# alanqrwang/nwhead

Hardware: AMD Instinct MI355X
Metric: query-predictions/sec (higher is better)
Workload: dtype f32; 1 GPU; K3 predict('full'): B=256 queries/step vs bank N=50000 d=512 C=200, bank sharded 1-way, 26 query batches coalesced per launch; B=256, N_support=50000, d=512, C=200, parallelism=support-shard x1

## Files before the change

nwhead_amd/csrc/fused_f16p.h:

```cpp
#pragma once
#include "fused_impl.h"
#include "persistent_pipe.h"

namespace nw {
namespace {

template <int RS, int QB, bool TWO = false>
struct PCfg : PipeCfg<16 * RS, 64 * QB, NCONS, NLOAD, TWO ? 3 : 4> {};

template <int RS, int KIND, int QB, int NCW = NCONS>
__device__ __forceinline__ void epilogue_p(f32x4 (&acc)[QB][RS], const float* hdr, int nrun, int2 bnd,
                                           const float* __restrict__ logit_scale, float* __restrict__ ws_m,
                                           float* __restrict__ ws_den, float* __restrict__ ws_num, int B, int N,
                                           int q0, int s0, int st, int wave, int lane
#ifdef NW_DIAG_FUSED
                                           , unsigned long long (&diag_)[8], unsigned long long& last_
#endif
                                           ) {
    using P = PCfg<RS, QB>;
    constexpr int BS = P::BS;
    constexpr bool NEED_NORM = (KIND != NW_SCORE_DOT);
    constexpr float L2E = 1.44269504088896340736f;
    typedef float f32x2 __attribute__((ext_vector_type(2)));
    const float* sn2 = hdr;
    const float* ssc = hdr + P::NH;
    const int* runid = reinterpret_cast<const int*>(hdr + 2 * P::NH);
    const float* qn2 = hdr + 3 * P::NH;
    const float* qsc_s = qn2 + 16 * QB * NCW;
    const int i = lane & 15, g = lane >> 4;
    float scale = 1.f;
    if (KIND == NW_SCORE_CLIP) scale = expf(*logit_scale);
    using SF = ScoreFactors<KIND>;
    float4 n4[RS], s4[RS];
#pragma unroll
    for (int r = 0; r < RS; ++r) {
        n4[r] = NEED_NORM ? *reinterpret_cast<const float4*>(sn2 + 16 * r + 4 * g) : make_float4(0.f, 0.f, 0.f, 0.f);
        s4[r] = *reinterpret_cast<const float4*>(ssc + 16 * r + 4 * g);
    }
    NW_PSTAMP(1);
    float4 K4[RS], B4[RS];
#pragma unroll
    for (int r = 0; r < RS; ++r) {
        SF::support(n4[r].x, s4[r].x, K4[r].x, B4[r].x);
        SF::support(n4[r].y, s4[r].y, K4[r].y, B4[r].y);
        SF::support(n4[r].z, s4[r].z, K4[r].z, B4[r].z);
        SF::support(n4[r].w, s4[r].w, K4[r].w, B4[r].w);
    }
#pragma unroll
    for (int j = 0; j < QB; ++j) {
        const int qrow = 16 * (QB * wave + j) + i;
        const int b = q0 + qrow;
        float Cq, Bq;
        SF::query(NEED_NORM ? qn2[qrow] : 0.f, qsc_s[qrow], scale, Cq, Bq);
        const f32x2 cq = {Cq, Cq}, bq = {Bq, Bq};
        float sc[RS][4];
#pragma unroll
        for (int r = 0; r < RS; ++r) {
            const f32x2 d01 = __builtin_elementwise_fma(f32x2{acc[j][r][0], acc[j][r][1]}, f32x2{K4[r].x, K4[r].y} * cq,
                                                        f32x2{B4[r].x, B4[r].y} + bq);
            const f32x2 d23 = __builtin_elementwise_fma(f32x2{acc[j][r][2], acc[j][r][3]}, f32x2{K4[r].z, K4[r].w} * cq,
                                                        f32x2{B4[r].z, B4[r].w} + bq);
            sc[r][0] = SF::finish_abs(d01.x);
            sc[r][1] = SF::finish_abs(d01.y);
            sc[r][2] = SF::finish_abs(d23.x);
            sc[r][3] = SF::finish_abs(d23.y);
        }
        NW_PSTAMP(2);
        constexpr float WORST = SF::DIST ? INFINITY : -INFINITY;
        if (s0 + BS > N) {
#pragma unroll
            for (int r = 0; r < RS; ++r)
#pragma unroll
                for (int e = 0; e < 4; ++e)
                    if (s0 + 16 * r + 4 * g + e >= N) sc[r][e] = WORST;
        }
        auto best = [](float a, float b) { return SF::DIST ? fminf(a, b) : fmaxf(a, b); };
        float mx[4] = {WORST, WORST, WORST, WORST};
#pragma unroll
        for (int r = 0; r < RS; ++r) mx[r & 3] = best(mx[r & 3], best(best(sc[r][0], sc[r][1]), best(sc[r][2], sc[r][3])));
        float ext = best(best(mx[0], mx[1]), best(mx[2], mx[3]));
        ext = SF::DIST ? group4_min(ext) : group4_max(ext);
        const float mloc = SF::DIST ? -ext : ext;
#pragma unroll
        for (int r = 0; r < RS; ++r)
#pragma unroll
            for (int e = 0; e < 4; ++e)
                sc[r][e] = __builtin_amdgcn_exp2f(SF::DIST ? ext - sc[r][e] : sc[r][e] - ext);
        NW_PSTAMP(3);
        float dloc;
        auto red4 = [](float x) { return group4_sum(x); };
        if (nrun <= 3) {
            float S0[2] = {0.f, 0.f}, S1[2] = {0.f, 0.f}, S2[2] = {0.f, 0.f};
            if (nrun == 1) {
#pragma unroll
                for (int r = 0; r < RS; ++r) {
                    S0[r & 1] += (sc[r][0] + sc[r][1]) + (sc[r][2] + sc[r][3]);
                }
            } else {
                const int b1 = bnd.x, b2 = (nrun == 3) ? bnd.y : BS;
                const float L1 = (float)(b1 - 4 * g);
                const float M2 = 1.f - (float)(b2 - 4 * g);
#pragma unroll
                for (int r = 0; r < RS; ++r) {
                    const int lo = 16 * r, hi = 16 * r + 16;
                    const bool in0 = hi <= b1, in2 = lo >= b2, in1 = lo >= b1 && hi <= b2;
                    const float quad = (sc[r][0] + sc[r][1]) + (sc[r][2] + sc[r][3]);
                    S0[r & 1] = __builtin_fmaf(in0 ? 1.f : 0.f, quad, S0[r & 1]);
                    S1[r & 1] = __builtin_fmaf(in1 ? 1.f : 0.f, quad, S1[r & 1]);
                    S2[r & 1] = __builtin_fmaf(in2 ? 1.f : 0.f, quad, S2[r & 1]);
                    if (!(in0 || in1 || in2)) {
#pragma unroll
                        for (int e = 0; e < 4; ++e) {
                            const float c = (float)(16 * r + e), ev = sc[r][e];
                            const float w1 = __builtin_amdgcn_fmed3f(L1 - c, 0.f, 1.f);
                            const float u2 = __builtin_amdgcn_fmed3f(c + M2, 0.f, 1.f);
                            S0[e & 1] = __builtin_fmaf(w1, ev, S0[e & 1]);
                            S2[e & 1] = __builtin_fmaf(u2, ev, S2[e & 1]);
                            S1[e & 1] = __builtin_fmaf((1.f - w1) - u2, ev, S1[e & 1]);
                        }
                    }
                }
            }
            const float s0v = red4(S0[0] + S0[1]);
            float s1v = 0.f, s2v = 0.f;
            if (nrun >= 2) s1v = red4(S1[0] + S1[1]);
            if (nrun == 3) s2v = red4(S2[0] + S2[1]);
            dloc = (s0v + s1v) + s2v;
            if (g == 0 && b < B) {
                ws_num[((size_t)st * BS) * B + b] = s0v;
                if (nrun >= 2) ws_num[((size_t)st * BS + 1) * B + b] = s1v;
                if (nrun == 3) ws_num[((size_t)st * BS + 2) * B + b] = s2v;
            }
        } else {
            float dl[4] = {0.f, 0.f, 0.f, 0.f};
#pragma unroll
            for (int r = 0; r < RS; ++r) dl[r & 3] += (sc[r][0] + sc[r][1]) + (sc[r][2] + sc[r][3]);
            dloc = red4((dl[0] + dl[1]) + (dl[2] + dl[3]));
            for (int run_base = 0; run_base < nrun; run_base += 16) {
                f32x4 Pm = {0.f, 0.f, 0.f, 0.f};
                const int want = run_base + i;
#pragma unroll
                for (int r = 0; r < RS; ++r) {
                    const int4 rid = *reinterpret_cast<const int4*>(runid + 16 * r + 4 * g);
                    Pm = __builtin_amdgcn_mfma_f32_16x16x4f32(rid.x == want ? 1.f : 0.f, sc[r][0], Pm, 0, 0, 0);
                    Pm = __builtin_amdgcn_mfma_f32_16x16x4f32(rid.y == want ? 1.f : 0.f, sc[r][1], Pm, 0, 0, 0);
                    Pm = __builtin_amdgcn_mfma_f32_16x16x4f32(rid.z == want ? 1.f : 0.f, sc[r][2], Pm, 0, 0, 0);
                    Pm = __builtin_amdgcn_mfma_f32_16x16x4f32(rid.w == want ? 1.f : 0.f, sc[r][3], Pm, 0, 0, 0);
                }
                if (b < B) {
#pragma unroll
                    for (int jj = 0; jj < 4; ++jj) {
                        const int run = run_base + 4 * g + jj;
                        if (run < nrun) ws_num[((size_t)st * BS + run) * B + b] = Pm[jj];
                    }
                }
            }
        }
        NW_PSTAMP(4);
        if (g == 0 && b < B) {
            ws_m[(size_t)st * B + b] = mloc;
            ws_den[(size_t)st * B + b] = dloc;
        }
        NW_PSTAMP(5);
    }
}

template <int RS, int KIND, bool TWO, int QB>
__global__ __launch_bounds__(TILE_THREADS, TWO ? 4 : 2) void nw_fused_f16p_kernel(
    const float* __restrict__ q, const float* __restrict__ s, const float* __restrict__ s_norm2,
    const float* __restrict__ s_scale, const float* __restrict__ q_norm2, const float* __restrict__ q_scale,
    const float* __restrict__ logit_scale, const int* __restrict__ ws_runid, const int* __restrict__ ws_nrun, const int* __restrict__ ws_bnd,
    float* __restrict__ ws_m, float* __restrict__ ws_den, float* __restrict__ ws_num, int B, int N, int d,
    int n_stiles, int n_qtiles, int qg) {
    using P = PCfg<RS, QB, TWO>;
    constexpr int BS = P::BS, BQP = P::BQP, TILE_F4 = P::TILE_F4, NB = P::NB;
    constexpr bool SINGLE = TWO || QB > 1;
    static_assert(!(TWO && QB > 1), "two 128-query workgroups do not fit the LDS of a CU");
    static_assert(P::THREADS == TILE_THREADS, "launch bounds");
    static_assert(RS == 8, "the persistent kernel is built for tiles of 128 supports");
    extern __shared__ __attribute__((aligned(16))) char smem[];
    float* hdr0 = reinterpret_cast<float*>(smem);
    float4* stage = reinterpret_cast<float4*>(smem + P::HDR_BYTES);

    const int tid = threadIdx.x, lane = tid & 63;
    const int wave = __builtin_amdgcn_readfirstlane(tid >> 6);
    const int nk = d / BK;
    const PersistentTiles tiles(blockIdx.x, gridDim.x, n_stiles, n_qtiles, qg);
    const int cu = tiles.cu, n_cu = tiles.n_cu, n_local = tiles.n_local;

    if (wave >= P::NCW) {
        persistent_loader<P>(tiles, wave - P::NCW, lane, hdr0, stage, q, s, s_norm2, s_scale, q_norm2, q_scale, ws_runid, B, N,
                             d);
    } else {
        const int i = lane & 15, g = lane >> 4;
        struct Frag {
            float4 bh[QB], bl[QB];
            float4 ah[RS], al[RS];
        };
        const int rsw = (i >> 1) & 7;
        auto load_frags = [&](Frag& f, int buf) {
            const float4* Qs = stage + ((unsigned)buf % NB) * TILE_F4;
            const float4* Ss = Qs + BQP * ROW_F4;
            const int sh = g ^ rsw, sl = (4 + g) ^ rsw;
#pragma unroll
            for (int j = 0; j < QB; ++j) {
                const int qrow = 16 * (QB * wave + j) + i;
                f.bh[j] = Qs[qrow * ROW_F4 + sh];
                f.bl[j] = Qs[qrow * ROW_F4 + sl];
            }
#pragma unroll
            for (int r = 0; r < RS; ++r) {
                f.ah[r] = Ss[(16 * r + i) * ROW_F4 + sh];
                f.al[r] = Ss[(16 * r + i) * ROW_F4 + sl];
            }
        };
        auto mm = [](const float4& a, const float4& b, f32x4 c) {
            return __builtin_amdgcn_mfma_f32_16x16x32_f16(__builtin_bit_cast(half8, a), __builtin_bit_cast(half8, b), c, 0, 0, 0);
        };
        f32x4 acc[QB][RS];
        auto mfma_stage = [&](const Frag& f) {
#pragma unroll
            for (int j = 0; j < QB; ++j)
#pragma unroll
                for (int r = 0; r < RS; ++r) acc[j][r] = mm(f.al[r], f.bh[j], acc[j][r]);
#pragma unroll
            for (int j = 0; j < QB; ++j)
#pragma unroll
                for (int r = 0; r < RS; ++r) acc[j][r] = mm(f.ah[r], f.bl[j], acc[j][r]);
#pragma unroll
            for (int j = 0; j < QB; ++j)
#pragma unroll
                for (int r = 0; r < RS; ++r) acc[j][r] = mm(f.ah[r], f.bh[j], acc[j][r]);
        };
        auto interleave = [&]() {
#pragma unroll
            for (int x = 0; x < 2 * (RS + 1); ++x) {
                __builtin_amdgcn_sched_group_barrier(0x008, 1, 0);
                __builtin_amdgcn_sched_group_barrier(0x100, 1, 0);
            }
            __builtin_amdgcn_sched_group_barrier(0x008, 3 * RS - 2 * (RS + 1), 0);
        };

        tile_barrier();
        int gi = 0;
        int par = 0;
#ifdef NW_DIAG_FUSED
        unsigned long long diag_[8] = {0, 0, 0, 0, 0, 0, 0, 0}, last_ = __builtin_amdgcn_s_memtime();
        const unsigned long long first_ = last_, first_rt_ = __builtin_amdgcn_s_memrealtime();
#endif
        for (int T = cu; T < n_local; T += n_cu) {
            int qt, st;
            tiles.decode(T, qt, st);
            const int q0 = qt * BQP, s0 = st * BS;
            const int nrun = ws_nrun[st];
            const int2 bnd = *reinterpret_cast<const int2*>(ws_bnd + 2 * (size_t)st);

#pragma unroll
            for (int j = 0; j < QB; ++j)
#pragma unroll
                for (int r = 0; r < RS; ++r) acc[j][r] = f32x4{0.f, 0.f, 0.f, 0.f};
            if constexpr (QB > 1) {
                struct F1 { float4 bh[QB]; float4 al[RS]; };
                struct F2 { float4 bl[QB]; float4 ah[RS]; };
                const int sh = g ^ rsw, sl = (4 + g) ^ rsw;
                const int qoff = (16 * QB * wave + i) * ROW_F4, soff = (BQP + i) * ROW_F4;
                auto stage_base = [&](int buf) { return stage + ((unsigned)buf % NB) * TILE_F4; };
                auto rd_bh = [&](const float4* S, int j) { return S[qoff + 16 * j * ROW_F4 + sh]; };
                auto rd_bl = [&](const float4* S, int j) { return S[qoff + 16 * j * ROW_F4 + sl]; };
                auto rd_ah = [&](const float4* S, int r) { return S[soff + 16 * r * ROW_F4 + sh]; };
                auto rd_al = [&](const float4* S, int r) { return S[soff + 16 * r * ROW_F4 + sl]; };
                auto pin = []() { __builtin_amdgcn_sched_barrier(0); };
                auto run_stage = [&](const F1& ac, F1& an, F2& b, int buf_next, auto has_next) {
#ifdef NW_ABL_NORD
                    constexpr bool NXT = false;
#else
                    constexpr bool NXT = decltype(has_next)::value;
#endif
                    const float4* Sn = stage_base(buf_next);
                    int n = 0;
#pragma unroll
                    for (int r = 0; r < RS; ++r)
#pragma unroll
                        for (int jx = 0; jx < QB; ++jx) {
                            const int j = (r & 1) ? QB - 1 - jx : jx;
                            acc[j][r] = mm(ac.al[r], ac.bh[j], acc[j][r]);
                            if (NXT && n < QB + RS) {
                                if (n < QB) an.bh[n] = rd_bh(Sn, n);
                                else an.al[n - QB] = rd_al(Sn, n - QB);
                            }
                            ++n;
                            pin();
                        }
#pragma unroll
                    for (int r = 0; r < RS; ++r)
#pragma unroll
                        for (int jx = 0; jx < QB; ++jx) {
                            const int j = (r & 1) ? QB - 1 - jx : jx;
                            acc[j][r] = mm(b.ah[r], b.bl[j], acc[j][r]);
                            pin();
                        }
                    if (NXT) {
#pragma unroll
                        for (int j = 0; j < QB; ++j) b.bl[j] = rd_bl(Sn, j);
                        pin();
                    }
#pragma unroll
                    for (int r = RS - 1; r >= 0; --r) {
#pragma unroll
                        for (int jx = 0; jx < QB; ++jx) {
                            const int j = (r & 1) ? jx : QB - 1 - jx;
                            acc[j][r] = mm(b.ah[r], ac.bh[j], acc[j][r]);
                        }
                        pin();
                        if (NXT) {
                            b.ah[r] = rd_ah(Sn, r);
                            pin();
                        }
                    }
                };
                using Yes = std::integral_constant<bool, true>;
                using No = std::integral_constant<bool, false>;
                F1 a0, a1;
                F2 b0;
                {
                    const float4* S0 = stage_base(gi);
#pragma unroll
                    for (int j = 0; j < QB; ++j) { a0.bh[j] = rd_bh(S0, j); b0.bl[j] = rd_bl(S0, j); }
#pragma unroll
                    for (int r = 0; r < RS; ++r) { a0.al[r] = rd_al(S0, r); b0.ah[r] = rd_ah(S0, r); }
#ifdef NW_ABL_NORD
                    a1 = a0;
#endif
                    pin();
                }
                int kt = 0;
                for (; kt + 2 < nk; kt += 2) {
                    run_stage(a0, a1, b0, gi + kt + 1, Yes{});
                    tile_barrier_nowait();
                    run_stage(a1, a0, b0, gi + kt + 2, Yes{});
                    tile_barrier_nowait();
                }
                if (kt + 2 == nk) {
                    run_stage(a0, a1, b0, gi + kt + 1, Yes{});
                    tile_barrier_nowait();
                    run_stage(a1, a0, b0, 0, No{});
                    tile_barrier_nowait();
                } else {
                    run_stage(a0, a1, b0, 0, No{});
                    tile_barrier_nowait();
                }
            } else if constexpr (SINGLE) {
                Frag f0;
                for (int kt = 0; kt < nk; ++kt) {
                    load_frags(f0, gi + kt);
                    mfma_stage(f0);
                    tile_barrier();
                }
            } else {
                Frag f0, f1;
                load_frags(f0, gi);
                int kt = 0;
                for (; kt + 2 < nk; kt += 2) {
                    load_frags(f1, gi + kt + 1);
                    mfma_stage(f0);
                    interleave();
                    tile_barrier();
                    load_frags(f0, gi + kt + 2);
                    mfma_stage(f1);
                    interleave();
                    tile_barrier();
                }
                for (; kt < nk; ++kt) {
                    if (kt + 1 < nk) load_frags(f1, gi + kt + 1);
                    mfma_stage(f0);
                    tile_barrier();
                    f0 = f1;
                }
            }
            gi += nk;
            NW_PSTAMP(0);
#ifndef NW_ABL_NOEPI
            epilogue_p<RS, KIND, QB>(acc, hdr0 + par * P::HDR_F, nrun, bnd, logit_scale, ws_m, ws_den, ws_num, B, N, q0, s0, st,
                                 wave, lane
#ifdef NW_DIAG_FUSED
                                 , diag_, last_
#endif
                                 );
#else
            keep_acc_alive(acc, ws_m, nrun, bnd);
#endif
            par = (par + 1 == P::NHB) ? 0 : par + 1;
            NW_PSTAMP(6);
        }
#ifdef NW_DIAG_FUSED
        diag_write_out(diag_, last_, first_, first_rt_);
#endif
    }
}

}
}
```

nwhead_amd/csrc/fused_f16p12.h:

```cpp
#pragma once
#include "fused_f16p.h"

namespace nw {
namespace {

struct P12 : PipeCfg<128, 256, 8, 4, 3> {
    static constexpr int RS = BS / 16, QB = BQP / (16 * NCW);
    static_assert(LDS_BYTES <= 160 * 1024, "LDS of one CU");
};

template <int KIND, bool CAND = false>
__device__ __forceinline__ void epilogue_p12(f32x4 (&acc)[P12::QB][P12::RS], const float* hdr, int nrun, int2 bnd,
                                             float scale, float* __restrict__ ws_m,
                                             float* __restrict__ ws_den, float* __restrict__ ws_num, int B, int N,
                                             int q0, int s0, int st, int wave, int lane, int n_stiles, int k
#ifdef NW_DIAG_FUSED
                                             , unsigned long long (&diag_)[8], unsigned long long& last_
#endif
                                             ) {
    using P = P12;
    constexpr int RS = P::RS, QB = P::QB, BS = P::BS;
    constexpr bool NEED_NORM = (KIND != NW_SCORE_DOT);
    typedef float f32x2 __attribute__((ext_vector_type(2)));
    const float* sn2 = hdr;
    const float* ssc = hdr + P::NH;
    const int* runid = reinterpret_cast<const int*>(hdr + 2 * P::NH);
    const float* qn2 = hdr + 3 * P::NH;
    const float* qsc_s = qn2 + P::BQP;
    const int i = lane & 15, g = lane >> 4;
    using SF = ScoreFactors<KIND>;
    float Cq[QB], Bq[QB];
#pragma unroll
    for (int j = 0; j < QB; ++j) {
        const int qrow = 16 * (QB * wave + j) + i;
        SF::query(NEED_NORM ? qn2[qrow] : 0.f, qsc_s[qrow], scale, Cq[j], Bq[j]);
    }
    NW_PSTAMP(1);
    float sc[QB][RS][4];
#pragma unroll
    for (int r = 0; r < RS; ++r) {
        const float4 n4 = NEED_NORM ? *reinterpret_cast<const float4*>(sn2 + 16 * r + 4 * g) : make_float4(0.f, 0.f, 0.f, 0.f);
        const float4 s4 = *reinterpret_cast<const float4*>(ssc + 16 * r + 4 * g);
        float4 K4, B4;
        SF::support(n4.x, s4.x, K4.x, B4.x);
        SF::support(n4.y, s4.y, K4.y, B4.y);
        SF::support(n4.z, s4.z, K4.z, B4.z);
        SF::support(n4.w, s4.w, K4.w, B4.w);
        float4 B4r = B4;
        asm volatile("" : "+v"(B4r.x), "+v"(B4r.y), "+v"(B4r.z), "+v"(B4r.w));
#pragma unroll
        for (int j = 0; j < QB; ++j) {
            const f32x2 cq = {Cq[j], Cq[j]}, bq = {Bq[j], Bq[j]};
            const float4 Bj = (j == 0) ? B4 : B4r;
            const f32x2 d01 = __builtin_elementwise_fma(f32x2{acc[j][r][0], acc[j][r][1]}, f32x2{K4.x, K4.y} * cq,
                                                        f32x2{Bj.x, Bj.y} + bq);
            const f32x2 d23 = __builtin_elementwise_fma(f32x2{acc[j][r][2], acc[j][r][3]}, f32x2{K4.z, K4.w} * cq,
                                                        f32x2{Bj.z, Bj.w} + bq);
            sc[j][r][0] = SF::finish_abs(d01.x);
            sc[j][r][1] = SF::finish_abs(d01.y);
            sc[j][r][2] = SF::finish_abs(d23.x);
            sc[j][r][3] = SF::finish_abs(d23.y);
            asm volatile("" : "+v"(sc[j][r][0]), "+v"(sc[j][r][1]), "+v"(sc[j][r][2]), "+v"(sc[j][r][3]));
        }
        __builtin_amdgcn_sched_barrier(0);
    }
    NW_PSTAMP(2);
    if constexpr (CAND) {
        int ln = lane;
        asm volatile("" : "+v"(ln));
        const int ci = ln & 15, cg = ln >> 4;
#pragma unroll
        for (int j = 0; j < QB; ++j) {
            float u[RS][4];
#pragma unroll
            for (int r = 0; r < RS; ++r)
#pragma unroll
                for (int e = 0; e < 4; ++e) u[r][e] = SF::DIST ? -sc[j][r][e] : sc[j][r][e];
            tile_candidates<RS>(u, reinterpret_cast<unsigned*>(ws_m), reinterpret_cast<int*>(ws_den), B, N,
                                q0 + 16 * (QB * wave + j) + ci, s0, cg, st, n_stiles, k);
            __builtin_amdgcn_sched_barrier(0);
        }
        return;
    }
    constexpr float WORST = SF::DIST ? INFINITY : -INFINITY;
    if (s0 + BS > N) {
        const int lim = N - s0 - 4 * g;
#pragma unroll
        for (int j = 0; j < QB; ++j)
#pragma unroll
            for (int r = 0; r < RS; ++r)
#pragma unroll
                for (int e = 0; e < 4; ++e)
                    if (16 * r + e >= lim) sc[j][r][e] = WORST;
    }
    auto best = [](float a, float b) { return SF::DIST ? fminf(a, b) : fmaxf(a, b); };
    auto best3 = [&](float a, float b, float c) { return best(best(a, b), c); };
    static_assert(RS == 8, "chain k takes the 16-row blocks k and k + 4");
    float ext[QB];
#pragma unroll
    for (int j = 0; j < QB; ++j) {
        float mx[4];
#pragma unroll
        for (int k = 0; k < 4; ++k) mx[k] = best3(sc[j][k][0], sc[j][k][1], sc[j][k][2]);
#pragma unroll
        for (int k = 0; k < 4; ++k) mx[k] = best3(mx[k], sc[j][k][3], sc[j][k + 4][0]);
#pragma unroll
        for (int k = 0; k < 4; ++k) mx[k] = best3(mx[k], sc[j][k + 4][1], sc[j][k + 4][2]);
#pragma unroll
        for (int k = 0; k < 4; ++k) mx[k] = best(mx[k], sc[j][k + 4][3]);
        ext[j] = best(best3(mx[0], mx[1], mx[2]), mx[3]);
    }
    group4_each(ext, best);
    float mloc[QB], dloc[QB], s0v[QB], s1v[QB] = {0.f, 0.f}, s2v[QB] = {0.f, 0.f};
#pragma unroll
    for (int j = 0; j < QB; ++j) {
        mloc[j] = SF::DIST ? -ext[j] : ext[j];
#pragma unroll
        for (int r = 0; r < RS; ++r)
#pragma unroll
            for (int e = 0; e < 4; ++e)
                sc[j][r][e] = __builtin_amdgcn_exp2f(SF::DIST ? ext[j] - sc[j][r][e] : sc[j][r][e] - ext[j]);
    }
    NW_PSTAMP(3);
    auto add = [](float a, float b) { return a + b; };
    if (nrun <= 3) {
        float S0[QB][2] = {{0.f, 0.f}, {0.f, 0.f}}, S1[QB][2] = {{0.f, 0.f}, {0.f, 0.f}}, S2[QB][2] = {{0.f, 0.f}, {0.f, 0.f}};
        if (nrun == 1) {
#pragma unroll
            for (int r = 0; r < RS; ++r)
#pragma unroll
                for (int j = 0; j < QB; ++j) S0[j][r & 1] += (sc[j][r][0] + sc[j][r][1]) + (sc[j][r][2] + sc[j][r][3]);
        } else {
            const int b1 = bnd.x, b2 = (nrun == 3) ? bnd.y : BS;
            const float L1 = (float)(b1 - 4 * g);
            const float M2 = 1.f - (float)(b2 - 4 * g);
#pragma unroll
            for (int r = 0; r < RS; ++r) {
                const int lo = 16 * r, hi = 16 * r + 16;
                const bool in0 = hi <= b1, in2 = lo >= b2, in1 = lo >= b1 && hi <= b2;
#pragma unroll
                for (int j = 0; j < QB; ++j) {
                    const float quad = (sc[j][r][0] + sc[j][r][1]) + (sc[j][r][2] + sc[j][r][3]);
                    S0[j][r & 1] = __builtin_fmaf(in0 ? 1.f : 0.f, quad, S0[j][r & 1]);
                    S1[j][r & 1] = __builtin_fmaf(in1 ? 1.f : 0.f, quad, S1[j][r & 1]);
                    S2[j][r & 1] = __builtin_fmaf(in2 ? 1.f : 0.f, quad, S2[j][r & 1]);
                }
                if (!(in0 || in1 || in2)) {
#pragma unroll
                    for (int e = 0; e < 4; ++e) {
                        const float c = (float)(16 * r + e);
                        const float w1 = __builtin_amdgcn_fmed3f(L1 - c, 0.f, 1.f);
                        const float u2 = __builtin_amdgcn_fmed3f(c + M2, 0.f, 1.f);
#pragma unroll
                        for (int j = 0; j < QB; ++j) {
                            const float ev = sc[j][r][e];
                            S0[j][e & 1] = __builtin_fmaf(w1, ev, S0[j][e & 1]);
                            S2[j][e & 1] = __builtin_fmaf(u2, ev, S2[j][e & 1]);
                            S1[j][e & 1] = __builtin_fmaf((1.f - w1) - u2, ev, S1[j][e & 1]);
                        }
                    }
                }
            }
        }
        if (nrun == 1) {
            float v[QB] = {S0[0][0] + S0[0][1], S0[1][0] + S0[1][1]};
            group4_each(v, add);
            s0v[0] = v[0], s0v[1] = v[1];
        } else if (nrun == 2) {
            float v[2 * QB] = {S0[0][0] + S0[0][1], S0[1][0] + S0[1][1], S1[0][0] + S1[0][1], S1[1][0] + S1[1][1]};
            group4_each(v, add);
            s0v[0] = v[0], s0v[1] = v[1], s1v[0] = v[2], s1v[1] = v[3];
        } else {
            float v[3 * QB] = {S0[0][0] + S0[0][1], S0[1][0] + S0[1][1], S1[0][0] + S1[0][1],
                               S1[1][0] + S1[1][1], S2[0][0] + S2[0][1], S2[1][0] + S2[1][1]};
            group4_each(v, add);
            s0v[0] = v[0], s0v[1] = v[1], s1v[0] = v[2], s1v[1] = v[3], s2v[0] = v[4], s2v[1] = v[5];
        }
#pragma unroll
        for (int j = 0; j < QB; ++j) dloc[j] = (s0v[j] + s1v[j]) + s2v[j];
    } else {
#pragma unroll
        for (int j = 0; j < QB; ++j) {
            float dl[4] = {0.f, 0.f, 0.f, 0.f};
#pragma unroll
            for (int r = 0; r < RS; ++r) dl[r & 3] += (sc[j][r][0] + sc[j][r][1]) + (sc[j][r][2] + sc[j][r][3]);
            dloc[j] = (dl[0] + dl[1]) + (dl[2] + dl[3]);
        }
        group4_each(dloc, add);
#pragma unroll
        for (int j = 0; j < QB; ++j) {
            const int b = q0 + 16 * (QB * wave + j) + i;
            for (int run_base = 0; run_base < nrun; run_base += 16) {
                f32x4 Pm = {0.f, 0.f, 0.f, 0.f};
                const int want = run_base + i;
#pragma unroll
                for (int r = 0; r < RS; ++r) {
                    const int4 rid = *reinterpret_cast<const int4*>(runid + 16 * r + 4 * g);
                    Pm = __builtin_amdgcn_mfma_f32_16x16x4f32(rid.x == want ? 1.f : 0.f, sc[j][r][0], Pm, 0, 0, 0);
                    Pm = __builtin_amdgcn_mfma_f32_16x16x4f32(rid.y == want ? 1.f : 0.f, sc[j][r][1], Pm, 0, 0, 0);
                    Pm = __builtin_amdgcn_mfma_f32_16x16x4f32(rid.z == want ? 1.f : 0.f, sc[j][r][2], Pm, 0, 0, 0);
                    Pm = __builtin_amdgcn_mfma_f32_16x16x4f32(rid.w == want ? 1.f : 0.f, sc[j][r][3], Pm, 0, 0, 0);
                }
                if (b < B) {
#pragma unroll
                    for (int jj = 0; jj < 4; ++jj) {
                        const int run = run_base + 4 * g + jj;
                        if (run < nrun) ws_num[((size_t)st * BS + run) * B + b] = Pm[jj];
                    }
                }
            }
        }
    }
    NW_PSTAMP(4);
    static_assert(QB == 2, "lane groups 0 / 1 carry query blocks 0 / 1, groups 2 / 3 the same blocks of the next array");
    int ln = lane;
    asm volatile("" : "+v"(ln));
    const int b = q0 + 16 * QB * wave + (ln & 31);
    const bool blk1 = ln & 16, arr1 = ln & 32;
    const size_t tb = (size_t)st * B + b, nb = (size_t)st * BS * B + b;
    if (b < B) {
        const float mv = blk1 ? mloc[1] : mloc[0], dv = blk1 ? dloc[1] : dloc[0];
        (arr1 ? ws_den : ws_m)[tb] = arr1 ? dv : mv;
        if (nrun <= 3) {
            const float n0 = blk1 ? s0v[1] : s0v[0], n1 = blk1 ? s1v[1] : s1v[0], n2 = blk1 ? s2v[1] : s2v[0];
            if (!arr1 || nrun >= 2) ws_num[nb + (arr1 ? B : 0)] = arr1 ? n1 : n0;
            if (!arr1 && nrun == 3) ws_num[nb + 2 * (size_t)B] = n2;
        }
    }
    NW_PSTAMP(5);
}

template <int KIND, bool HALF = false, bool CAND = false>
__global__ __launch_bounds__(P12::THREADS, 3) void nw_fused_f16p_kernel_w12(
    const float* __restrict__ q, const float* __restrict__ s, const float* __restrict__ s_norm2,
    const float* __restrict__ s_scale, const float* __restrict__ q_norm2, const float* __restrict__ q_scale,
    const float* __restrict__ logit_scale, const int* __restrict__ ws_runid, const int* __restrict__ ws_nrun,
    const int* __restrict__ ws_bnd, float* __restrict__ ws_m, float* __restrict__ ws_den, float* __restrict__ ws_num, int B,
    int N, int d, int n_stiles, int n_qtiles, int qg, int k) {
    static_assert(!CAND || HALF, "the candidate form exists for half-precision rows only");
    using P = P12;
    constexpr int RS = P::RS, QB = P::QB, BS = P::BS, BQP = P::BQP, NB = P::NB;
    extern __shared__ __attribute__((aligned(16))) char smem[];
    float* hdr0 = reinterpret_cast<float*>(smem);
    float4* stage = reinterpret_cast<float4*>(smem + P::HDR_BYTES);

    const int tid = threadIdx.x, lane = tid & 63;
    const int wave = __builtin_amdgcn_readfirstlane(tid >> 6);
    const int nk = d / BK;
    const PersistentTiles tiles(blockIdx.x, gridDim.x, n_stiles, n_qtiles, qg);
    const int cu = tiles.cu, n_cu = tiles.n_cu, n_local = tiles.n_local;

    if (wave >= P::NCW) {
        persistent_loader<P, !CAND>(tiles, wave - P::NCW, lane, hdr0, stage, q, s, s_norm2, s_scale, q_norm2, q_scale, ws_runid, B, N,
                             d);
    } else {
        const int i = lane & 15, g = lane >> 4;
        const int rsw = (i >> 1) & 7;
        const int sh = g ^ rsw, sl = (4 + g) ^ rsw;
        const int qoff = (16 * QB * wave + i) * ROW_F4, soff = (BQP + i) * ROW_F4;
        struct QF { float4 bh[QB], bl[QB]; };
        struct SW { float4 al[2], ah[2]; };
        constexpr int NW_ = RS / 2;
#ifdef NW_DIAG_FUSED
        unsigned long long diag_[8] = {0, 0, 0, 0, 0, 0, 0, 0}, last_ = 0;
#endif
#ifdef NW_DIAG_HEAD
        unsigned long long h0_ = 0, h1_ = 0;
#define NW_HEAD_STAMP(t) asm volatile("s_memtime %0" : "=s"(t))
#else
#define NW_HEAD_STAMP(t)
#endif
        auto mm = [](const float4& a, const float4& b, f32x4 c) {
            return __builtin_amdgcn_mfma_f32_16x16x32_f16(__builtin_bit_cast(half8, a), __builtin_bit_cast(half8, b), c, 0, 0, 0);
        };
        auto pin = []() { __builtin_amdgcn_sched_barrier(0); };
        f32x4 acc[QB][RS];
        constexpr int NM = HALF ? 8 : 12;
        auto mm_1 = [&](const SW& w, const QF& f, int p, int m) {
            const int ph = m >> 2, x = (m >> 1) & 1, j = m & 1;
            const float4& a = HALF ? (ph == 0 ? w.ah[x] : w.al[x]) : (ph == 0 ? w.al[x] : w.ah[x]);
            const float4& b = HALF ? (ph == 0 ? f.bh[j] : f.bl[j]) : (ph == 1 ? f.bl[j] : f.bh[j]);
            acc[j][2 * p + x] = mm(a, b, acc[j][2 * p + x]);
        };
        auto mm_w = [&](const SW& w, const QF& f, int p, auto&& behind) {
#pragma unroll
            for (int m = 0; m < NM; ++m) {
                mm_1(w, f, p, m);
                behind(m);
            }
            pin();
        };
        auto nothing = [](int) {};
        typedef const __attribute__((address_space(3))) f32x4 lds_f4;
        const unsigned ring0 = (unsigned)(uintptr_t)(__attribute__((address_space(3))) char*)(char*)stage;
        unsigned a_qh = ring0 + 16u * (qoff + sh), a_ql = ring0 + 16u * (qoff + sl);
        unsigned a_sh = ring0 + 16u * (soff + sh), a_sl = ring0 + 16u * (soff + sl);
        asm volatile("" : "+v"(a_qh), "+v"(a_ql), "+v"(a_sh), "+v"(a_sl));
        auto lds_rd = [](unsigned a, int f4) { return __builtin_bit_cast(float4, *(lds_f4*)(uintptr_t)(a + 16u * f4)); };
        auto q_h = [&](int j) { return lds_rd(a_qh, 16 * j * ROW_F4); };
        auto q_l = [&](int j) { return lds_rd(a_ql, 16 * j * ROW_F4); };
        auto s_h = [&](int blk) { return lds_rd(a_sh, 16 * blk * ROW_F4); };
        auto s_l = [&](int blk) { return lds_rd(a_sl, 16 * blk * ROW_F4); };
        auto advance = [&](int slot, int m) {
            const unsigned step = (slot + 1 == NB) ? 0u - (unsigned)((NB - 1) * P::TILE_F4 * 16) : (unsigned)(P::TILE_F4 * 16);
            unsigned& a = (m == 0) ? a_qh : (m == 1) ? a_ql : (m == 2) ? a_sh : a_sl;
            a += step;
            asm volatile("" : "+v"(a));
        };
        SW wa, wb;
        auto rd_first = [&](QF& f, SW& w, int n) {
            const bool qlo = n >= 4, slo = (n < 4) != HALF;
            const int r = n & 3;
            if (r == 0 || r == 3) {
                const int x = r == 3;
                if (slo) w.al[x] = s_l(x);
                else w.ah[x] = s_h(x);
            } else {
                if (qlo) f.bl[r - 1] = q_l(r - 1);
                else f.bh[r - 1] = q_h(r - 1);
            }
        };
        auto rd_pair = [&](SW& w, int p, int n) {
            const int x = n & 1;
            if ((n < 2) != HALF) w.al[x] = s_l(2 * p + x);
            else w.ah[x] = s_h(2 * p + x);
        };
        auto run_stage = [&](const QF& fp, QF& fc, int slot, auto first) {
            constexpr bool FIRST = decltype(first)::value;
#ifdef NW_ABL_NORD
            constexpr bool RD = FIRST;
#else
            constexpr bool RD = true;
#endif
            if constexpr (FIRST) {
#pragma unroll
                for (int n = 0; n < 8; ++n) {
                    rd_first(fc, wa, n);
                    pin();
                }
            } else {
                NW_HEAD_STAMP(h0_);
                mm_w(wb, fp, NW_ - 1, [&](int m) {
                    if (m == 0) NW_HEAD_STAMP(h1_);
                    if (m < 8) {
                        pin();
                        if (RD) rd_first(fc, wa, m);
                        pin();
                    }
                });
            }
#pragma unroll
            for (int p = 0; p + 1 < NW_; ++p) {
                SW& wr = (p & 1) ? wa : wb;
                mm_w((p & 1) ? wb : wa, fc, p, [&](int m) {
                    if (m < 4) {
                        pin();
                        if (RD) rd_pair(wr, p + 1, m);
                        pin();
                    } else if (p + 2 == NW_ && m < 8) {
                        pin();
                        advance(slot, m - 4);
                        pin();
                    }
                });
            }
            static_assert(NW_ % 2 == 0, "the last pair of a stage sits in wb");
            tile_barrier();
#ifdef NW_DIAG_HEAD
            if (!FIRST) diag_[6] += h1_ - h0_;
#endif
        };
        using Yes = std::integral_constant<bool, true>;
        using No = std::integral_constant<bool, false>;

        float scale = 1.f;
        if (KIND == NW_SCORE_CLIP)
            scale = __builtin_bit_cast(float, __builtin_amdgcn_readfirstlane(__builtin_bit_cast(int, expf(*logit_scale))));
        tile_barrier();
        int gi = 0;
        int par = 0;
        auto next_slot = [&]() {
            const int b = gi;
            gi = (gi + 1 == NB) ? 0 : gi + 1;
            return b;
        };
#ifdef NW_DIAG_FUSED
        last_ = __builtin_amdgcn_s_memtime();
        const unsigned long long first_ = last_, first_rt_ = __builtin_amdgcn_s_memrealtime();
#endif
        for (int T = cu; T < n_local; T += n_cu) {
            int qt, st;
            tiles.decode(T, qt, st);
            const int q0 = qt * BQP, s0 = st * BS;
            int nrun = 0;
            int2 bnd = {0, 0};
            if constexpr (!CAND) {
                nrun = ws_nrun[st];
                bnd = *reinterpret_cast<const int2*>(ws_bnd + 2 * (size_t)st);
            }
#pragma unroll
            for (int j = 0; j < QB; ++j)
#pragma unroll
                for (int r = 0; r < RS; ++r) acc[j][r] = f32x4{0.f, 0.f, 0.f, 0.f};
            QF f0, f1;
#ifdef NW_ABL_NORD
#pragma unroll
            for (int n = 0; n < 8; ++n) rd_first(f1, wa, n);
#endif
            run_stage(f1, f0, next_slot(), Yes{});
            int kt = 1;
            for (; kt + 1 < nk; kt += 2) {
                run_stage(f0, f1, next_slot(), No{});
                run_stage(f1, f0, next_slot(), No{});
            }
            if (kt < nk) {
                run_stage(f0, f1, next_slot(), No{});
                mm_w(wb, f1, NW_ - 1, nothing);
            } else {
                mm_w(wb, f0, NW_ - 1, nothing);
            }
            NW_PSTAMP(0);
#ifndef NW_ABL_NOEPI
            epilogue_p12<KIND, CAND>(acc, hdr0 + par * P::HDR_F, nrun, bnd, scale, ws_m, ws_den, ws_num, B, N, q0, s0, st, wave,
                                     lane, n_stiles, k
#ifdef NW_DIAG_FUSED
                                     , diag_, last_
#endif
                                     );
#else
            keep_acc_alive(acc, ws_m, nrun, bnd);
#endif
            par = (par + 1 == P::NHB) ? 0 : par + 1;
#ifndef NW_DIAG_HEAD
            NW_PSTAMP(6);
#endif
        }
#ifdef NW_DIAG_FUSED
        diag_write_out(diag_, last_, first_, first_rt_);
#endif
    }
}

}
}
```

nwhead_amd/csrc/persistent_pipe.h:

```cpp
#pragma once
#include "tile_core.h"

namespace nw {
namespace {

#ifdef NW_DIAG_FUSED
__device__ unsigned long long nw_diag_p[8 * 1024];
__device__ unsigned long long nw_diag_rt[2 * 1024];
#define NW_PSTAMP(k)                                                                         \
    do {                                                                                     \
        unsigned long long now_;                                                             \
        __builtin_amdgcn_sched_barrier(0);                                                   \
        asm volatile("s_memtime %0\n\ts_waitcnt lgkmcnt(0)" : "=s"(now_)::"memory");         \
        __builtin_amdgcn_sched_barrier(0);                                                   \
        diag_[k] += now_ - last_;                                                            \
        last_ = now_;                                                                        \
    } while (0)

__device__ __forceinline__ void diag_write_out(const unsigned long long (&diag_)[8], unsigned long long last_,
                                               unsigned long long first_, unsigned long long first_rt_) {
    if (threadIdx.x == 0 && blockIdx.x < 1024) {
        for (int k = 0; k < 7; ++k) nw_diag_p[8 * blockIdx.x + k] = diag_[k];
        nw_diag_p[8 * blockIdx.x + 7] = last_ - first_;
        nw_diag_rt[2 * blockIdx.x] = first_rt_;
        nw_diag_rt[2 * blockIdx.x + 1] = __builtin_amdgcn_s_memrealtime();
    }
}
#else
#define NW_PSTAMP(k)
#endif

template <int QB, int RS>
__device__ __forceinline__ void keep_acc_alive(const f32x4 (&acc)[QB][RS], float* ws_m, int nrun, int2 bnd) {
    f32x4 sum_ = {0.f, 0.f, 0.f, 0.f};
    for (int j = 0; j < QB; ++j)
        for (int r = 0; r < RS; ++r) sum_ += acc[j][r];
    if (sum_[0] + sum_[1] + sum_[2] + sum_[3] == 12345.678f) ws_m[threadIdx.x] = sum_[0] + nrun + bnd.x;
}

template <int BS_, int BQP_, int NCW_, int NLW_, int NB_>
struct PipeCfg {
    static constexpr int BS = BS_, BQP = BQP_, NCW = NCW_, NLW = NLW_;
    static constexpr int THREADS = 64 * (NCW + NLW);
    static constexpr int NB = NB_;
    static constexpr int AHEAD = NB - 1;
    static constexpr int TILE_F4 = (BQP + BS) * ROW_F4;
    static constexpr int NT = (BQP + BS) / 8;
    static constexpr int NI = NT / NLW;
    static constexpr int NQI = BQP / 8 / NLW;
    static constexpr int N64 = (BS + 63) / 64;
    static constexpr int NH = N64 * 64;
    static constexpr int HDR_F = 3 * NH + 2 * BQP;
    static constexpr int NP = 3 * N64 + 2 * (BQP / 64);
    static constexpr int HPW = (NP + NLW - 1) / NLW;
    static constexpr int NHB = 3;
    static constexpr size_t HDR_BYTES = (size_t)NHB * HDR_F * 4;
    static constexpr size_t LDS_BYTES = HDR_BYTES + (size_t)NB * TILE_F4 * 16;
    static_assert(NT % NLW == 0, "every loader wave issues the same number of pieces");
    static_assert(BQP % (8 * NLW) == 0, "query and support pieces must not share a loader round");
    static_assert(HDR_BYTES % 16 == 0, "stage buffers must stay 16-byte aligned");
    static_assert(NI + HPW < 64, "vmcnt is a 6-bit field");
};

struct PersistentTiles {
    int xcd, cu, n_cu;
    int n_qtiles, qg;
    int ns_x;
    int n_full;
    int nq_x;
    int n_local;
    int grp_tiles;
    __device__ __forceinline__ PersistentTiles(unsigned block, unsigned grid, int n_stiles, int n_qtiles_, int qg_)
        : xcd(block & 7), cu(block >> 3), n_cu(grid >> 3), n_qtiles(n_qtiles_), qg(qg_) {
        ns_x = n_stiles >> 3;
        n_full = ns_x * n_qtiles;
        const int rem = n_stiles & 7;
        nq_x = (n_qtiles - xcd + 7) >> 3;
        n_local = n_full + rem * nq_x;
        grp_tiles = qg * ns_x;
    }
    __device__ __forceinline__ void decode(int L, int& qt, int& st) const {
        if (L >= n_full) {
            const int r = L - n_full, j = r / nq_x;
            st = 8 * ns_x + j;
            qt = xcd + 8 * (r - j * nq_x);
            return;
        }
        const int gi = L / grp_tiles, r = L - gi * grp_tiles;
        const int g = min(qg, n_qtiles - gi * qg);
        const int stl = r / g;
        qt = gi * qg + (r - stl * g);
        st = stl * 8 + xcd;
    }
};

template <class P, bool RUNID = true>
__device__ __forceinline__ void persistent_loader(const PersistentTiles& tiles, int lw, int lane, float* hdr0, float4* stage,
                                                  const float* __restrict__ q, const float* __restrict__ s,
                                                  const float* __restrict__ s_norm2, const float* __restrict__ s_scale,
                                                  const float* __restrict__ q_norm2, const float* __restrict__ q_scale,
                                                  const int* __restrict__ ws_runid, int B, int N, int d) {
    constexpr int BS = P::BS, BQP = P::BQP, NI = P::NI, NLW = P::NLW;
    const int nk = d / BK;
    const int n_local = tiles.n_local, n_cu = tiles.n_cu;
    unsigned voff[NI];
    int iT = tiles.cu, ikt = 0, irot = 0, ipar = 0;
    int iq0 = 0, is0 = 0, ist = 0;
    int gs = 0;
    auto set_tile = [&](int T) {
        int qt, st;
        tiles.decode(T, qt, st);
        iq0 = qt * BQP;
        is0 = st * BS;
        ist = st;
        irot = st % nk;
#pragma unroll
        for (int m = 0; m < NI; ++m) {
            const int R = 8 * (lw + NLW * m) + (lane >> 3);
            const int lslot = (lane & 7) ^ ((R >> 1) & 7);
            const int rel = (m < P::NQI) ? min(iq0 + R, B - 1) - iq0 : min(is0 + R - BQP, N - 1) - is0;
            voff[m] = ((unsigned)rel * (unsigned)d + lslot * 4) * 4u;
        }
    };
    auto dma4 = [&](const void* src, float* dst) {
        __builtin_amdgcn_global_load_lds((const __attribute__((address_space(1))) void*)src,
                                         (__attribute__((address_space(3))) void*)dst, 4, 0, 0);
    };
    auto issue_header = [&]() {
        float* h = hdr0 + ipar * P::HDR_F;
#pragma unroll
        for (int k = 0; k < P::HPW; ++k) {
            const int pc = min(lw + NLW * k, P::NP - 1);
            if (pc < 3 * P::N64) {
                const int arr = pc / P::N64, c = pc - arr * P::N64;
                const int row = is0 + 64 * c + lane;
                float* dst = h + arr * P::NH + 64 * c;
                if (arr == 0) dma4(s_norm2 + min(row, N - 1), dst);
                else if (arr == 1) dma4(s_scale + min(row, N - 1), dst);
                else if constexpr (RUNID) dma4(ws_runid + (size_t)ist * BS + 64 * c + lane, dst);
                else dma4(s_scale + min(row, N - 1), h + P::NH + 64 * c);
            } else {
                const int qp = pc - 3 * P::N64, arr = qp / (BQP / 64), c = qp - arr * (BQP / 64);
                const int row = min(iq0 + 64 * c + lane, B - 1);
                dma4((arr == 0 ? q_norm2 : q_scale) + row, h + 3 * P::NH + arr * BQP + 64 * c);
            }
        }
    };
    bool young_hdr = false;
    auto issue_next = [&]() {
        if (iT >= n_local) return false;
        int kc = ikt + irot;
        if (kc >= nk) kc -= nk;
        float4* buf = stage + gs * P::TILE_F4;
        const char* qb = reinterpret_cast<const char*>(q + (size_t)iq0 * d) + (size_t)kc * BK * 4;
        const char* sb = reinterpret_cast<const char*>(s + (size_t)is0 * d) + (size_t)kc * BK * 4;
#ifndef NW_ABL_NODMA
#pragma unroll
        for (int m = 0; m < NI; ++m) {
            const char* g = ((m < P::NQI) ? qb : sb) + voff[m];
            __builtin_amdgcn_global_load_lds((const __attribute__((address_space(1))) void*)g,
                                             (__attribute__((address_space(3))) void*)(buf + 64 * (lw + NLW * m)), 16, 0, 0);
        }
#else
        (void)qb; (void)sb; (void)buf;
#endif
        young_hdr = (ikt == 0);
        if (young_hdr) issue_header();
        gs = (gs + 1 == P::NB) ? 0 : gs + 1;
        if (++ikt == nk) {
            ikt = 0;
            ipar = (ipar + 1 == P::NHB) ? 0 : ipar + 1;
            iT += n_cu;
            if (iT < n_local) set_tile(iT);
        }
        return true;
    };
#ifndef NW_ABL_NODMA
    constexpr int YOUNG = NI;
#else
    constexpr int YOUNG = 0;
#endif
    auto wait_landed = [&](bool issued) {
        if (!issued) wait_vmcnt<0>();
        else if (young_hdr) wait_vmcnt<YOUNG + P::HPW>();
        else wait_vmcnt<YOUNG>();
    };
    if (iT < n_local) set_tile(iT);
    bool more = true;
#pragma unroll
    for (int k0 = 0; k0 < P::AHEAD; ++k0) more = issue_next();
    wait_landed(more);
    tile_barrier();
    for (int T = tiles.cu; T < n_local; T += n_cu) {
        for (int kt = 0; kt < nk; ++kt) {
            more = issue_next();
            wait_landed(more);
            tile_barrier();
        }
    }
}

}
}
```

Before: 7.757 million query-predictions/s.

## Pass tile metadata through LDS records and prefetch next tile's first fragments

The loader wave now reads each tile's run count and bounds from global memory and writes them, together with the query offset and support tile index, into a small LDS record next to the header. Consumer waves read that record after the MMA loop instead of decoding the tile and loading ws_nrun/ws_bnd from global at the start of each tile. In the p12 kernel, the main loop is restructured so that when nk is even, the first few fragment reads of the next tile are interleaved into the last MFMA stage of the current tile. The intent is to hide per-tile global latency and the pipeline bubble at tile boundaries. The cost is extra LDS, an inline-asm write, and a packed 16-bit bounds encoding that assumes the bounds fit in 16 bits.

```diff
diff --git a/nwhead_amd/csrc/fused_f16p.h b/nwhead_amd/csrc/fused_f16p.h
--- a/nwhead_amd/csrc/fused_f16p.h
+++ b/nwhead_amd/csrc/fused_f16p.h
@@ -178,7 +178,9 @@
     static_assert(!(TWO && QB > 1), "two 128-query workgroups do not fit the LDS of a CU");
     static_assert(P::THREADS == TILE_THREADS, "launch bounds");
     static_assert(RS == 8, "the persistent kernel is built for tiles of 128 supports");
+    static_assert((TWO ? 2 : 1) * P::LDS_TOTAL <= 160 * 1024, "LDS of one CU (TWO: of half a CU)");
     extern __shared__ __attribute__((aligned(16))) char smem[];
+    __shared__ __attribute__((aligned(P::REC_BYTES))) i32x4 rec0[P::REC_BYTES / 16];
     float* hdr0 = reinterpret_cast<float*>(smem);
     float4* stage = reinterpret_cast<float4*>(smem + P::HDR_BYTES);
 
@@ -189,8 +191,8 @@
     const int cu = tiles.cu, n_cu = tiles.n_cu, n_local = tiles.n_local;
 
     if (wave >= P::NCW) {
-        persistent_loader<P>(tiles, wave - P::NCW, lane, hdr0, stage, q, s, s_norm2, s_scale, q_norm2, q_scale, ws_runid, B, N,
-                             d);
+        persistent_loader<P>(tiles, wave - P::NCW, lane, hdr0, rec0, stage, q, s, s_norm2, s_scale, q_norm2, q_scale, ws_runid,
+                             ws_nrun, ws_bnd, B, N, d);
     } else {
         const int i = lane & 15, g = lane >> 4;
         struct Frag {
@@ -249,11 +251,6 @@
         const unsigned long long first_ = last_, first_rt_ = __builtin_amdgcn_s_memrealtime();
 #endif
         for (int T = cu; T < n_local; T += n_cu) {
-            int qt, st;
-            tiles.decode(T, qt, st);
-            const int q0 = qt * BQP, s0 = st * BS;
-            const int nrun = ws_nrun[st];
-            const int2 bnd = *reinterpret_cast<const int2*>(ws_bnd + 2 * (size_t)st);
 
 #pragma unroll
             for (int j = 0; j < QB; ++j)
@@ -378,6 +375,9 @@
                 }
             }
             gi += nk;
+            const TileRec rec = uniform_tile_rec(load_tile_rec(rec0 + par));
+            const int q0 = rec.q0, st = rec.st, s0 = st * BS, nrun = rec.nrun;
+            const int2 bnd = rec.bnd;
             NW_PSTAMP(0);
 #ifndef NW_ABL_NOEPI
             epilogue_p<RS, KIND, QB>(acc, hdr0 + par * P::HDR_F, nrun, bnd, logit_scale, ws_m, ws_den, ws_num, B, N, q0, s0, st,
diff --git a/nwhead_amd/csrc/fused_f16p12.h b/nwhead_amd/csrc/fused_f16p12.h
--- a/nwhead_amd/csrc/fused_f16p12.h
+++ b/nwhead_amd/csrc/fused_f16p12.h
@@ -6,7 +6,7 @@
 
 struct P12 : PipeCfg<128, 256, 8, 4, 3> {
     static constexpr int RS = BS / 16, QB = BQP / (16 * NCW);
-    static_assert(LDS_BYTES <= 160 * 1024, "LDS of one CU");
+    static_assert(LDS_TOTAL <= 160 * 1024, "LDS of one CU");
 };
 
 template <int KIND, bool CAND = false>
@@ -241,6 +241,7 @@
     using P = P12;
     constexpr int RS = P::RS, QB = P::QB, BS = P::BS, BQP = P::BQP, NB = P::NB;
     extern __shared__ __attribute__((aligned(16))) char smem[];
+    __shared__ __attribute__((aligned(P::REC_BYTES))) i32x4 rec0[P::REC_BYTES / 16];
     float* hdr0 = reinterpret_cast<float*>(smem);
     float4* stage = reinterpret_cast<float4*>(smem + P::HDR_BYTES);
 
@@ -251,8 +252,8 @@
     const int cu = tiles.cu, n_cu = tiles.n_cu, n_local = tiles.n_local;
 
     if (wave >= P::NCW) {
-        persistent_loader<P, !CAND>(tiles, wave - P::NCW, lane, hdr0, stage, q, s, s_norm2, s_scale, q_norm2, q_scale, ws_runid, B, N,
-                             d);
+        persistent_loader<P, !CAND>(tiles, wave - P::NCW, lane, hdr0, rec0, stage, q, s, s_norm2, s_scale, q_norm2, q_scale,
+                                    ws_runid, ws_nrun, ws_bnd, B, N, d);
     } else {
         const int i = lane & 15, g = lane >> 4;
         const int rsw = (i >> 1) & 7;
@@ -269,6 +270,12 @@
 #define NW_HEAD_STAMP(t) asm volatile("s_memtime %0" : "=s"(t))
 #else
 #define NW_HEAD_STAMP(t)
+#endif
+#ifdef NW_DIAG_TILE
+        unsigned long long t0_ = 0, tile1_ = 0, ntile_ = 0;
+#define NW_TILE_STAMP(t) asm volatile("s_memtime %0\n\ts_waitcnt lgkmcnt(0)" : "=s"(t)::"memory")
+#else
+#define NW_TILE_STAMP(t)
 #endif
         auto mm = [](const float4& a, const float4& b, f32x4 c) {
             return __builtin_amdgcn_mfma_f32_16x16x32_f16(__builtin_bit_cast(half8, a), __builtin_bit_cast(half8, b), c, 0, 0, 0);
@@ -325,7 +332,8 @@
             if ((n < 2) != HALF) w.al[x] = s_l(2 * p + x);
             else w.ah[x] = s_h(2 * p + x);
         };
-        auto run_stage = [&](const QF& fp, QF& fc, int slot, auto first) {
+        constexpr int NEARLY = 6;
+        auto run_stage = [&](const QF& fp, QF& fc, int slot, auto first, bool pre = false) {
             constexpr bool FIRST = decltype(first)::value;
 #ifdef NW_ABL_NORD
             constexpr bool RD = FIRST;
@@ -333,8 +341,15 @@
             constexpr bool RD = true;
 #endif
             if constexpr (FIRST) {
-#pragma unroll
-                for (int n = 0; n < 8; ++n) {
+                if (!pre) {
+#pragma unroll
+                    for (int n = 0; n < NEARLY; ++n) {
+                        rd_first(fc, wa, n);
+                        pin();
+                    }
+                }
+#pragma unroll
+                for (int n = NEARLY; n < 8; ++n) {
                     rd_first(fc, wa, n);
                     pin();
                 }
@@ -353,6 +368,7 @@
             for (int p = 0; p + 1 < NW_; ++p) {
                 SW& wr = (p & 1) ? wa : wb;
                 mm_w((p & 1) ? wb : wa, fc, p, [&](int m) {
+                    if (FIRST && p == 0 && m == 0) NW_TILE_STAMP(t0_);
                     if (m < 4) {
                         pin();
                         if (RD) rd_pair(wr, p + 1, m);
@@ -368,6 +384,16 @@
             tile_barrier();
 #ifdef NW_DIAG_HEAD
             if (!FIRST) diag_[6] += h1_ - h0_;
+#endif
+#ifdef NW_DIAG_TILE
+            if (FIRST) {
+                unsigned long long t1_;
+                NW_TILE_STAMP(t1_);
+                diag_[6] += t0_ - last_;
+                last_ = t0_;
+                tile1_ += t1_ - t0_;
+                ++ntile_;
+            }
 #endif
         };
         using Yes = std::integral_constant<bool, true>;
@@ -388,37 +414,52 @@
         last_ = __builtin_amdgcn_s_memtime();
         const unsigned long long first_ = last_, first_rt_ = __builtin_amdgcn_s_memrealtime();
 #endif
+#ifdef NW_ABL_NORD
+        constexpr bool EARLY = false;
+#else
+        constexpr bool EARLY = !CAND;
+#endif
+        const bool nk_even = !(nk & 1);
+        bool pre = false;
+        QF f0, f1;
         for (int T = cu; T < n_local; T += n_cu) {
-            int qt, st;
-            tiles.decode(T, qt, st);
-            const int q0 = qt * BQP, s0 = st * BS;
-            int nrun = 0;
-            int2 bnd = {0, 0};
-            if constexpr (!CAND) {
-                nrun = ws_nrun[st];
-                bnd = *reinterpret_cast<const int2*>(ws_bnd + 2 * (size_t)st);
-            }
 #pragma unroll
             for (int j = 0; j < QB; ++j)
 #pragma unroll
                 for (int r = 0; r < RS; ++r) acc[j][r] = f32x4{0.f, 0.f, 0.f, 0.f};
-            QF f0, f1;
 #ifdef NW_ABL_NORD
 #pragma unroll
             for (int n = 0; n < 8; ++n) rd_first(f1, wa, n);
 #endif
-            run_stage(f1, f0, next_slot(), Yes{});
-            int kt = 1;
+            run_stage(f1, f0, next_slot(), Yes{}, pre);
+            run_stage(f0, f1, next_slot(), No{});
+            int kt = 2;
             for (; kt + 1 < nk; kt += 2) {
+                run_stage(f1, f0, next_slot(), No{});
                 run_stage(f0, f1, next_slot(), No{});
+            }
+            i32x4 recv;
+            pre = EARLY && nk_even && T + n_cu < n_local;
+            if (kt < nk) {
                 run_stage(f1, f0, next_slot(), No{});
-            }
-            if (kt < nk) {
-                run_stage(f0, f1, next_slot(), No{});
-                mm_w(wb, f1, NW_ - 1, nothing);
+                recv = load_tile_rec(rec0 + par);
+                mm_w(wb, f0, NW_ - 1, nothing);
             } else {
-                mm_w(wb, f0, NW_ - 1, nothing);
-            }
+                recv = load_tile_rec(rec0 + par);
+                if (pre)
+                    mm_w(wb, f1, NW_ - 1, [&](int m) {
+                        if (m < NEARLY) {
+                            pin();
+                            rd_first(f0, wa, m);
+                            pin();
+                        }
+                    });
+                else
+                    mm_w(wb, f1, NW_ - 1, nothing);
+            }
+            const TileRec rec = uniform_tile_rec(recv);
+            const int q0 = rec.q0, st = rec.st, s0 = st * BS, nrun = rec.nrun;
+            const int2 bnd = rec.bnd;
             NW_PSTAMP(0);
 #ifndef NW_ABL_NOEPI
             epilogue_p12<KIND, CAND>(acc, hdr0 + par * P::HDR_F, nrun, bnd, scale, ws_m, ws_den, ws_num, B, N, q0, s0, st, wave,
@@ -437,6 +478,9 @@
         }
 #ifdef NW_DIAG_FUSED
         diag_write_out(diag_, last_, first_, first_rt_);
+#ifdef NW_DIAG_TILE
+        if (threadIdx.x == 0 && blockIdx.x < 1024) nw_diag_t[2 * blockIdx.x] = tile1_, nw_diag_t[2 * blockIdx.x + 1] = ntile_;
+#endif
 #endif
     }
 }
diff --git a/nwhead_amd/csrc/persistent_pipe.h b/nwhead_amd/csrc/persistent_pipe.h
--- a/nwhead_amd/csrc/persistent_pipe.h
+++ b/nwhead_amd/csrc/persistent_pipe.h
@@ -26,6 +26,9 @@
         nw_diag_rt[2 * blockIdx.x + 1] = __builtin_amdgcn_s_memrealtime();
     }
 }
+#ifdef NW_DIAG_TILE
+__device__ unsigned long long nw_diag_t[2 * 1024];
+#endif
 #else
 #define NW_PSTAMP(k)
 #endif
@@ -56,6 +59,9 @@
     static constexpr int NHB = 3;
     static constexpr size_t HDR_BYTES = (size_t)NHB * HDR_F * 4;
     static constexpr size_t LDS_BYTES = HDR_BYTES + (size_t)NB * TILE_F4 * 16;
+    static constexpr size_t REC_BYTES = 1024;
+    static_assert(NHB * 16 <= REC_BYTES, "the records fit their block");
+    static constexpr size_t LDS_TOTAL = LDS_BYTES + REC_BYTES;
     static_assert(NT % NLW == 0, "every loader wave issues the same number of pieces");
     static_assert(BQP % (8 * NLW) == 0, "query and support pieces must not share a loader round");
     static_assert(HDR_BYTES % 16 == 0, "stage buffers must stay 16-byte aligned");
@@ -94,18 +100,45 @@
     }
 };
 
+typedef int i32x4 __attribute__((ext_vector_type(4)));
+struct TileRec {
+    int q0, st, nrun;
+    int2 bnd;
+};
+__device__ __forceinline__ void write_tile_rec(i32x4* rec, int q0, int st, int nrun, int2 bnd) {
+    const unsigned a = (unsigned)(uintptr_t)(__attribute__((address_space(3))) char*)(char*)rec;
+    const i32x4 v = {q0, st, nrun, (int)(((unsigned)bnd.x & 0xffffu) | ((unsigned)bnd.y << 16))};
+    asm volatile("ds_write_b128 %0, %1\n\ts_nop 1" ::"v"(a), "v"(v) : "memory");
+}
+__device__ __forceinline__ i32x4 load_tile_rec(const i32x4* rec) {
+    return *(const __attribute__((address_space(3))) i32x4*)rec;
+}
+__device__ __forceinline__ TileRec uniform_tile_rec(const i32x4& v) {
+    TileRec t;
+    t.q0 = __builtin_amdgcn_readfirstlane(v.x);
+    t.st = __builtin_amdgcn_readfirstlane(v.y);
+    t.nrun = __builtin_amdgcn_readfirstlane(v.z);
+    const int b = __builtin_amdgcn_readfirstlane(v.w);
+    t.bnd = make_int2(b & 0xffff, (int)((unsigned)b >> 16));
+    return t;
+}
+
 template <class P, bool RUNID = true>
-__device__ __forceinline__ void persistent_loader(const PersistentTiles& tiles, int lw, int lane, float* hdr0, float4* stage,
+__device__ __forceinline__ void persistent_loader(const PersistentTiles& tiles, int lw, int lane, float* hdr0, i32x4* rec0,
+                                                  float4* stage,
                                                   const float* __restrict__ q, const float* __restrict__ s,
                                                   const float* __restrict__ s_norm2, const float* __restrict__ s_scale,
                                                   const float* __restrict__ q_norm2, const float* __restrict__ q_scale,
-                                                  const int* __restrict__ ws_runid, int B, int N, int d) {
+                                                  const int* __restrict__ ws_runid, const int* __restrict__ ws_nrun,
+                                                  const int* __restrict__ ws_bnd, int B, int N, int d) {
     constexpr int BS = P::BS, BQP = P::BQP, NI = P::NI, NLW = P::NLW;
     const int nk = d / BK;
     const int n_local = tiles.n_local, n_cu = tiles.n_cu;
     unsigned voff[NI];
     int iT = tiles.cu, ikt = 0, irot = 0, ipar = 0;
     int iq0 = 0, is0 = 0, ist = 0;
+    int inrun = 0;
+    int2 ibnd = {0, 0};
     int gs = 0;
     auto set_tile = [&](int T) {
         int qt, st;
@@ -114,6 +147,12 @@
         is0 = st * BS;
         ist = st;
         irot = st % nk;
+        if constexpr (RUNID) {
+            if (lw == 0) {
+                inrun = ws_nrun[st];
+                ibnd = *reinterpret_cast<const int2*>(ws_bnd + 2 * (size_t)st);
+            }
+        }
 #pragma unroll
         for (int m = 0; m < NI; ++m) {
             const int R = 8 * (lw + NLW * m) + (lane >> 3);
@@ -145,6 +184,7 @@
                 dma4((arr == 0 ? q_norm2 : q_scale) + row, h + 3 * P::NH + arr * BQP + 64 * c);
             }
         }
+        if (lw == 0 && lane == 0) write_tile_rec(rec0 + ipar, iq0, ist, inrun, ibnd);
     };
     bool young_hdr = false;
     auto issue_next = [&]() {
```

After: 7.797 million query-predictions/s, median of 6. Within noise of the previous version (+0.5%).
